# ChristianSteger/HORAYZON

Measured on AMD Instinct MI355X. Metric: grid_cells_per_s (horizon_gridded, 360 azimuths, 3601^2 SRTM-like tile), higher is better.
Workload: dtype f32

## Files before the change

### horayzon_amd/csrc/hz_api.hip

```cpp
#include "hz_internal.h"
#include <cmath>
#include <cstring>
#include <cstdlib>
#include <string>
#include <vector>
#include <limits>
#include <mutex>
#include <utility>
#include <thread>
#include <atomic>

namespace hz {

static thread_local std::string g_error;

int set_error(int code, const char *fmt, ...) {
    char buf[1024];
    va_list ap;
    va_start(ap, fmt);
    vsnprintf(buf, sizeof(buf), fmt, ap);
    va_end(ap);
    g_error = buf;
    return code;
}
// ... 400 lines not shown
    if (hipEventCreate(&n0) != hipSuccess || hipEventCreate(&n1) != hipSuccess) {
        if (n0) (void)hipEventDestroy(n0);
        return set_error(HZ_ERR_HIP, "hipEventCreate failed");
    }
    (void)hipEventRecord(n0, st);
    const int rc = near_launch(sc, na, st);
    (void)hipEventRecord(n1, st);
    if (!rc) {
        (void)hipEventSynchronize(n1);
        float mn = 0.0f;
        (void)hipEventElapsedTime(&mn, n0, n1);
        *ms_near += mn;
    }
    (void)hipEventDestroy(n0); (void)hipEventDestroy(n1);
    return rc;
}

static int plan_leftover(const Scene *sc, const hz_opts *opts, int rows_max, int dim_in_1, int left_t[HZ_LEFT_LEVELS], HorizonArgs &a) {
    int n_left_launches = 0;
    for (int l = 0; l < HZ_LEFT_LEVELS; l++) left_t[l] = 0;
    const int pack = opts ? opts->left_min : 0;
    const unsigned upack = pack == 0 ? HZ_LEFT_DEFAULT : (pack < 0 ? 0u : (unsigned)pack);
    for (int l = 0; l < HZ_LEFT_LEVELS; l++) {
        left_t[l] = (int)std::min((upack >> (8 * l)) & 0xffu, 56u);
        if (left_t[l] == 0) break;
        n_left_launches = l + 1;
    }
    if ((opts && opts->count_work) || n_left_launches == 0) return 0;
    const TileMap tm = make_tile_map((rows_max + 15) / 16, (dim_in_1 + 15) / 16);
    unsigned long long units = (unsigned long long)tm.per_xcd * 8ull * 4ull;
    unsigned long long total = 0, cap_max = 0;
    for (int l = 0; l < n_left_launches; l++) {
        unsigned long long cap = ((units * (unsigned long long)left_t[l] + 63ull) & ~63ull) + 64ull;
        if (opts && opts->left_cap_test > 0) cap = std::min<unsigned long long>(cap, ((unsigned long long)opts->left_cap_test + 63ull) & ~63ull);
        a.left_base[l] = (unsigned)total; a.left_cap[l] = (unsigned)cap;
        total += cap; cap_max = std::max(cap_max, cap);
        units = cap / 64ull;
    }
    const size_t rec_bytes = (size_t)total * HZ_LEFT_WORDS * sizeof(unsigned);
    const size_t sort_words = 4 * (size_t)cap_max + sort_temp_elems((size_t)cap_max) + 64;
    const size_t need = rec_bytes + sort_words * sizeof(uint32_t);
    if (total >= (1ull << 31) || (unsigned long long)rows_max * (unsigned long long)dim_in_1 >= 0xffffffffull) return 0;
    if (sc->left_bytes < need) {
        if (sc->left_buf) (void)hipFree(sc->left_buf);
        sc->left_buf = nullptr; sc->left_bytes = 0;
        if (hipMalloc(&sc->left_buf, need) != hipSuccess) { (void)hipGetLastError(); sc->left_buf = nullptr; return 0; }
        sc->left_bytes = need;
// ... 117 lines not shown
    a.mid_idx = d_mid.dev;
    a.top_nodes = opts ? opts->top_nodes : -1;
    a.regroup = opts ? opts->regroup : -1;
    a.count_work = opts ? opts->count_work : 0;
    a.hit_cache = (opts && opts->no_hit_cache) ? 0 : 1;
    a.counters = (unsigned long long *)cnt_dev;
    const int near_opt = opts ? opts->no_near_skip : 0;
    const bool height_field = (sc->hdr.flags & HZ_BLOB_HEIGHT_FIELD) != 0;
    const bool bad_map = (sc->hdr.flags & HZ_BLOB_BAD_MAP) != 0;
    const bool use_near = near_opt <= 0 && (height_field || bad_map || near_opt < 0) &&
                          azim_num <= near_max_azim() && tb.elev_num <= 65534;
    a.near_idx = nullptr; a.near_r = nullptr; a.scratch_row = nullptr;
    a.tile_list = nullptr; a.n_list = 0;
    const int verify_n = (opts && opts->verify_near > 0) ? opts->verify_near : 0;
    a.verify_near = (opts && opts->count_work) ? verify_n : 0;
    float ms_near = 0.0f;

    unsigned long long cnt[16] = {0}, n_verified = 0, n_mon_violations = 0;
    NearMonitor mon;
    float ms = 0.0f, ms_svf = 0.0f;
    int fallbacks = 0;
    unsigned long long redo_blocks = 0, redo_groups = 0;

    struct Ev { hipEvent_t a = nullptr, b = nullptr, c = nullptr, d = nullptr, l = nullptr; };
    std::vector<Ev> evs;
    std::vector<size_t> ev_of;
    hipStream_t st_copy = nullptr;
    auto free_events = [&]() {
        for (auto &e : evs) {
            if (e.a) (void)hipEventDestroy(e.a);
            if (e.b) (void)hipEventDestroy(e.b);
            if (e.c) (void)hipEventDestroy(e.c);
            if (e.d) (void)hipEventDestroy(e.d);
            if (e.l) (void)hipEventDestroy(e.l);
        }
        if (st_copy) { stream_release(sc->device, st_copy); st_copy = nullptr; }
    };
    if (stream_out && (rc = stream_acquire(sc->device, &st_copy))) return rc;
    if (use_near) {
        const size_t cells = (size_t)std::min(chunk_rows, row_end - row_begin) * dim_in_1;
        const size_t need = ((cells * (size_t)azim_num * 2 + 255) & ~(size_t)255) + cells * 4;
        if (sc->near_bytes < need) {
            if (sc->near_buf) (void)hipFree(sc->near_buf);
            sc->near_buf = nullptr; sc->near_bytes = 0;
            if (hipMalloc(&sc->near_buf, need) != hipSuccess) { free_events(); return set_error(HZ_ERR_HIP, "hipMalloc of the near-field certificates failed"); }
            sc->near_bytes = need;
        }
    }
    int left_t[HZ_LEFT_LEVELS];
    const int n_left_launches = plan_leftover(sc, opts, std::min(chunk_rows, row_end - row_begin), dim_in_1, left_t, a);
    a.left_min = n_left_launches > 0 ? left_t[0] : 0;
    a.left_rec = n_left_launches > 0 ? (unsigned *)sc->left_buf : nullptr;
    a.left_regroup = (opts && (opts->left_tune & 0xff) > 0) ? (opts->left_tune & 0xff) : HZ_LEFT_REGROUP;
    a.left_key_shift = (opts && ((opts->left_tune >> 8) & 0xff) > 0) ? std::min(((opts->left_tune >> 8) & 0xff) - 1, 8) : HZ_LEFT_KEY_SHIFT;
    a.persist_grid = (opts && opts->persist_grid > 0) ? opts->persist_grid : 0;
    a.no_persist = (opts && opts->persist_grid < 0) ? 1 : 0;
    unsigned *near_reasons = nullptr;
    struct ReasonsFree { unsigned **p; ~ReasonsFree() { if (*p) (void)hipFree(*p); } } reasons_free{&near_reasons};
    if (use_near && opts && opts->verbose >= 2) {
        if (hipMalloc((void **)&near_reasons, 20 * sizeof(unsigned)) != hipSuccess) { (void)hipGetLastError(); near_reasons = nullptr; }
        else (void)hipMemsetAsync(near_reasons, 0, 20 * sizeof(unsigned), st);
    }
    HostPinner pinner;
    if (stream_out && !(opts && opts->no_host_pin)) {
        std::vector<size_t> cb;
        for (int rb = row_begin; rb < row_end; rb += chunk_rows) cb.push_back((size_t)(std::min(rb + chunk_rows, row_end) - rb) * row_bytes);
        pinner.start(sc->device, reinterpret_cast<char *>(hori_slab_host), cb);
    }
    auto copy_out = [&](int k) -> int {
        const int rb = row_begin + k * chunk_rows, re = std::min(rb + chunk_rows, row_end);
        const void *src = (k & 1) ? tmp_hori2 : tmp_hori;
        Ev &e = evs[ev_of[(size_t)k]];
        char *dst = reinterpret_cast<char *>(hori_row0 + (size_t)rb * dim_in_1 * azim_num);
        const size_t bytes = (size_t)(re - rb) * row_bytes;
        std::vector<size_t> cuts;
        if (!pinner.planned.empty()) cuts = pinner.cuts_for(dst, bytes);
        cuts.push_back(bytes);
// ... 35 lines not shown
        }
        {
            Ev e;
            if (hipEventCreate(&e.a) != hipSuccess || hipEventCreate(&e.b) != hipSuccess || hipEventCreate(&e.c) != hipSuccess ||
                hipEventCreate(&e.d) != hipSuccess) {
                evs.push_back(e);
                return fail(set_error(HZ_ERR_HIP, "hipEventCreate failed"));
            }
            evs.push_back(e);
            ev_of.push_back(evs.size() - 1);
            if (hipMemcpyAsync(cnt_dev, zeros, sizeof(zeros), hipMemcpyHostToDevice, st) != hipSuccess)
                return fail(set_error(HZ_ERR_HIP, "counter reset failed"));
            if (stream_out && n_chunk >= 2) (void)hipStreamWaitEvent(st, evs[ev_of[(size_t)n_chunk - 2]].d, 0);
            a.level_stack = (sc->level_stack.load(std::memory_order_relaxed) != 0 || (opts && opts->level_stack > 0)) ? 1
                            : ((opts && opts->level_stack < 0) ? opts->level_stack : 0);
            (void)hipEventRecord(e.a, st);
            if (verify_n > 0 && !a.count_work && use_near) {
                if ((rc = mon.launch(sc, a, verify_n, rb, st))) return fail(rc);
            }
            auto launch_chunk = [&](int *safe_out) -> int {
                int r = horizon_launch(sc, a, st, safe_out);
                if (r || n_left_launches == 0) return r;
                if (!evs.back().l && hipEventCreate(&evs.back().l) != hipSuccess) return set_error(HZ_ERR_HIP, "hipEventCreate failed");
                (void)hipEventRecord(evs.back().l, st);
                for (int l = 1; l <= n_left_launches && !r; l++) {
                    if ((r = left_sort(a, l - 1, st))) break;
                    HorizonArgs b = a;
                    b.left_mode = l; b.left_min = l < n_left_launches ? left_t[l] : 0;
                    if (n_left_launches > 1) b.level_stack = 1;
                    b.tile_list = nullptr; b.n_list = 0;
                    r = horizon_launch(sc, b, st, nullptr);
                }
                return r;
            };
            int safe = 0;
            rc = launch_chunk(&safe);
            if (!rc && !safe) {
                unsigned long long cov[32] = {0};
                if (hipMemcpyAsync(cov, cnt_dev, sizeof(cov), hipMemcpyDeviceToHost, st) != hipSuccess ||
                    hipStreamSynchronize(st) != hipSuccess)
                    return fail(set_error(HZ_ERR_HIP, "horizon kernel failed: %s", hipGetErrorString(hipGetLastError())));
                const unsigned long long ov = cov[8], lov = cov[30];
                if (ov != 0 || lov != 0) {
                    const unsigned long long tiles = (unsigned long long)((re - rb + 7) / 8) * (unsigned long long)((dim_in_1 + 7) / 8);
                    fallbacks++;
                    a.level_stack = 1;
                    if (ov <= HZ_REDO_CAP && lov <= HZ_REDO_CAP && (ov + lov) * 4 <= tiles) {
                        redo_blocks += ov + lov; redo_groups += lov;
                        if (ov != 0) {
                            a.tile_list = reinterpret_cast<const int *>((unsigned long long *)cnt_dev + HZ_CNT_N);
                            a.n_list = (int)ov;
                            rc = horizon_launch(sc, a, st, &safe);
                            a.tile_list = nullptr; a.n_list = 0;
                        }
                        if (!rc && lov != 0) {
                            HorizonArgs b = a;
                            b.left_mode = 1; b.left_min = 0;
                            b.tile_list = reinterpret_cast<const int *>((unsigned long long *)cnt_dev + HZ_CNT_N) + HZ_REDO_CAP;
                            b.n_list = (int)lov;
                            rc = horizon_launch(sc, b, st, nullptr);
                        }
                    } else {
                        sc->level_stack.store(1, std::memory_order_relaxed);
                        if (hipMemcpyAsync(cnt_dev, zeros, sizeof(zeros), hipMemcpyHostToDevice, st) != hipSuccess)
                            return fail(set_error(HZ_ERR_HIP, "counter reset failed"));
                        (void)hipEventRecord(e.a, st);
                        rc = launch_chunk(&safe);
                    }
                }
            }
            if (!rc && mon.active) rc = mon.collect(st, &n_verified, &n_mon_violations);
            (void)hipEventRecord(e.b, st);
            if (!rc && want_topo) {
                const size_t o = (size_t)(rb - row_begin) * dim_in_1;
                const float *tilt_chunk = tilt0 ? tilt0 + 3 * (size_t)rb * dim_in_1 : nullptr;
                if (!want_vsf && !want_open)
                    rc = svf_launch(d_azim.dev, hori_chunk, tilt_chunk, re - rb, dim_in_1, azim_num, d_svf.dev + o, st);
                else
                    rc = topo_multi_launch(d_azim.dev, hori_chunk, tilt_chunk, re - rb, dim_in_1, azim_num,
                                           want_svf ? d_svf.dev + o : nullptr, want_vsf ? d_vsf.dev + o : nullptr,
                                           want_open ? d_open.dev + o : nullptr, st);
            }
            (void)hipEventRecord(e.c, st);
            if (!rc && stream_out && n_chunk >= 1) rc = copy_out(n_chunk - 1);
            if (rc) return fail(rc);
            unsigned long long c[HZ_CNT_N];
            if (hipMemcpyAsync(c, cnt_dev, sizeof(c), hipMemcpyDeviceToHost, st) != hipSuccess ||
                hipStreamSynchronize(st) != hipSuccess)
                return fail(set_error(HZ_ERR_HIP, "horizon kernel failed: %s", hipGetErrorString(hipGetLastError())));
            float m1 = 0.0f, m2 = 0.0f;
            (void)hipEventElapsedTime(&m1, e.a, e.b);
            (void)hipEventElapsedTime(&m2, e.b, e.c);
            ms += m1; ms_svf += m2;
            if (evs.back().l) { float m3 = 0.0f; (void)hipEventElapsedTime(&m3, evs.back().l, e.b); ms_left += m3; }
            for (int k = 0; k < 16; k++) cnt[k] += c[k];
            left_cells += c[28]; left_again += c[29];
            n_verified += c[21];
            if (a.count_work && opts && opts->verbose >= 3) {
                const unsigned long long t0 = ~c[20];
                fprintf(stderr, "hz xcd spans [ms] rows %d..%d:", rb, re);
                for (int x = 0; x < 8; x++) fprintf(stderr, " %.1f", c[12 + x] ? (double)(c[12 + x] - t0) * 1.0e-5 : 0.0);
                fprintf(stderr, "\n");
            }
        }
    }
    Timer t_d2h; t_d2h.start();
    if (stream_out) {
        rc = copy_out(n_chunk - 1);
        const hipError_t se = hipStreamSynchronize(st_copy);
        pinner.finish();
        if (!rc && se != hipSuccess) rc = set_error(HZ_ERR_HIP, "copy of the horizon failed: %s", hipGetErrorString(se));
        if (rc) { free_events(); return rc; }
    }
    free_events();
    HZ_HIP(hipGetLastError());
    if ((rc = d_hori.finish(st))) return rc;
    if ((rc = d_svf.finish(st))) return rc;
// ... 423 lines not shown
    const size_t bytes = (n ? n : 1) * 4;
    HZ_HIP(hipMalloc(&di, bytes)); HZ_HIP(hipMalloc(&dout, bytes)); HZ_HIP(hipMalloc(&tmp, scan_temp_elems(n) * 4 + 16));
    HZ_HIP(hipMemcpy(di, in, n * 4, hipMemcpyHostToDevice));
    rc = exclusive_scan_u32((const uint32_t *)di, (uint32_t *)dout, n, (uint32_t *)tmp, st);
    if (!rc) {
        HZ_HIP(hipStreamSynchronize(st));
        HZ_HIP(hipMemcpy(out, dout, n * 4, hipMemcpyDeviceToHost));
    }
    (void)hipFree(di); (void)hipFree(dout); (void)hipFree(tmp);
    return rc;
}

int hz_debug_valu_peak(int device, int packed, int waves_per_simd, double *winst_per_s_per_simd,
                       double *clock_ghz, int *simds) {
    int rc = select_device(device);
    if (rc) return rc;
    return bench_valu_peak(packed, waves_per_simd, winst_per_s_per_simd, clock_ghz, simds);
}

int hz_debug_set(const char *key, int value) {
    if (!key) return hz::set_error(HZ_ERR_ARG, "hz_debug_set: null key");
    if (!strcmp(key, "shadow_fast_cap")) hz::g_shadow_fast_cap.store(value < 0 ? HZ_SHADOW_FAST_CAP_DEFAULT : value, std::memory_order_relaxed);
    else if (!strcmp(key, "topo_wide")) hz::g_topo_wide.store(value != 0, std::memory_order_relaxed);
    else if (!strcmp(key, "accum_chunk")) hz::g_accum_chunk.store(value < 0 ? 0 : value, std::memory_order_relaxed);
    else return hz::set_error(HZ_ERR_ARG, "hz_debug_set: unknown key '%s'", key);
    return HZ_OK;
}

int hz_debug_inst_rate(int device, int op, double *cycles_per_inst) {
    int rc = select_device(device);
    if (rc) return rc;
    return bench_inst_rate(op, cycles_per_inst);
}

int hz_debug_copy_peak(int device, size_t bytes, double *gbs) {
    int rc = select_device(device);
    if (rc) return rc;
    return bench_copy_peak(bytes, gbs);
}

static int slope_api(int which, const float *x, const float *y, const float *z, int len_0, int len_1,
                     const float *rot_mat, int output_rot, float *vec_tilt, int device) {
    if (!x || !y || !z || !vec_tilt) return set_error(HZ_ERR_ARG, "NULL argument");
    if (len_0 <= 0 || len_1 <= 0) return set_error(HZ_ERR_ARG, "Inconsistent shapes / number of dimensions of input arrays");
    if (which == 1 && output_rot && !rot_mat) return set_error(HZ_ERR_ARG, "'rot_mat' must be provided for 'output_rot = True'");
    int rc = select_device(device);
// ... 544 lines not shown
```

### horayzon_amd/csrc/hz_horizon.hip

```cpp
#include "hz_search.h"
#include <vector>

namespace hz {

#ifndef HZ_TPB
#define HZ_TPB 256
#endif
#define HZ_WPB (HZ_TPB / 64)
#ifndef HZ_QLEN
#define HZ_QLEN 2
#endif

struct HorizonParams {
    SceneView sv;
    Tables tb;
    const float *vec_norm, *vec_north;
    const uint8_t *mask;
    float *hori;
    int offset_0, offset_1, dim_in_1;
    int row_begin, row_end;
    TileMap tm;
    float dist, hori_fill, ray_org_elev;
    float dist_box, neg_tau;
    int top_nodes, regroup, stack_bytes, leaf_bias, stage_bytes, hit_cache, stack_cap;
    int pre_bytes;
    const unsigned short *near_idx;
    const float *near_r;
    float *scratch_row;
    int verify_near;
    unsigned verify_mask;
    unsigned long long *counters;
    const int *tile_list;
    int n_list;
    int *redo_list;
    int left_min, left_mode;
    unsigned left_in_base;
    unsigned left_out_base, left_out_cap;
    unsigned *left_rec, *left_in_ctl, *left_out_ctl;
    const unsigned *left_perm;
    int persist;
    unsigned *queue;
};

__device__ __forceinline__ void hz_left_write(unsigned *w, unsigned cert, unsigned k, unsigned flags,
                                                        unsigned ind, unsigned prev, unsigned pazim, unsigned count, float lim_up, float lim_low,
                                                        float elev_samp, float ev, unsigned cache, float st0, float st1, float st2) {
    w[0] = cert;
    w[1] = k; w[2] = flags; w[3] = ind; w[4] = prev; w[5] = pazim; w[6] = count;
    w[7] = __float_as_uint(lim_up); w[8] = __float_as_uint(lim_low); w[9] = __float_as_uint(elev_samp); w[10] = __float_as_uint(ev);
    w[11] = cache; w[12] = __float_as_uint(st0); w[13] = __float_as_uint(st1); w[14] = __float_as_uint(st2); w[15] = 0u;
}

template <int ALG, bool COUNT, bool STAGE, bool NODELET, bool LEVELSTACK, bool LEFT = false>
#ifndef HZ_WG_PER_CU
#define HZ_WG_PER_CU 5
#endif
__global__ __launch_bounds__(HZ_TPB, (COUNT ? 4 : HZ_WG_PER_CU) * (4 / HZ_WPB)) void k_horizon(HorizonParams p_arg) {
    typedef const __attribute__((address_space(4))) HorizonParams *hz_kparams;
    hz_kparams pk = (hz_kparams)__builtin_amdgcn_kernarg_segment_ptr();
#if defined(__HIP_DEVICE_COMPILE__)
#define HZ_LOAD_PARAMS(dst) dst = *pk
#else
#define HZ_LOAD_PARAMS(dst) dst = p_arg
#endif
    HorizonParams p;
    HZ_LOAD_PARAMS(p);
    extern __shared__ __attribute__((aligned(16))) unsigned char smem[];
    int *stack = reinterpret_cast<int *>(smem + p.pre_bytes);
    const float4 *top = reinterpret_cast<const float4 *>(smem + p.pre_bytes + p.stack_bytes);
    const int tid = threadIdx.x;
    const int ntop = p.top_nodes;
    if (NODELET && ntop > 0) {
        float4 *dst = reinterpret_cast<float4 *>(smem + p.pre_bytes + p.stack_bytes);
        const float4 *src = reinterpret_cast<const float4 *>(p.sv.nodes);
        for (int i = tid; i < ntop * 2; i += HZ_TPB) dst[i] = src[i];
        __syncthreads();
    }

    const int wave = __builtin_amdgcn_readfirstlane(tid >> 6);
    const int xcc_own = (int)(__builtin_amdgcn_s_getreg((3 << 11) | 20) & 7u);
    int xcc_off = 0;
    int left_on = 1;
  for (;;) {
    asm volatile("" : "+s"(pk));
    HZ_LOAD_PARAMS(p);
    int tid_b = tid;
    asm volatile("" : "+v"(tid_b));
    const int lane = tid_b & 63;
#define HZ_KEEP(x) asm volatile("" : "+s"(x))
    HZ_KEEP(p.leaf_bias); HZ_KEEP(p.regroup); HZ_KEEP(p.neg_tau); HZ_KEEP(p.sv.cx); HZ_KEEP(p.sv.cy); HZ_KEEP(p.sv.cz);
    HZ_KEEP(p.near_idx); HZ_KEEP(p.near_r);
#undef HZ_KEEP
    int ti = 0, tj = 0;
    int blk = (int)blockIdx.x * HZ_WPB + wave;
    unsigned rec0 = 0u, rec_n = 0u;
    if (LEFT) {
        blk = -1;
        const unsigned groups = (p.left_in_ctl[1] + 63u) / 64u;
        if (p.tile_list) {
            const int b = (int)blockIdx.x * HZ_WPB + wave;
            const int g = b < p.n_list ? p.tile_list[b] : -1;
            if (g >= 0 && (unsigned)g < groups) { blk = g; rec0 = (unsigned)g * 64u; rec_n = min(64u, p.left_in_ctl[1] - (unsigned)g * 64u); }
        } else
        while (xcc_off < 8) {
            const unsigned x = (unsigned)((xcc_own + xcc_off) & 7);
            unsigned q = 0u;
            if (lane == 0) q = atomicAdd(&p.left_in_ctl[8 + x], 1u);
            q = (unsigned)__builtin_amdgcn_readfirstlane((int)q);
            const unsigned g = (((q >> 5) * 8u + x) << 5) | (q & 31u);
            if (g < groups) { blk = (int)g; rec0 = g * 64u; rec_n = min(64u, p.left_in_ctl[1] - g * 64u); break; }
            xcc_off++;
        }
        if (blk < 0) break;
    } else if (p.persist) {
        blk = -1;
        while (xcc_off < 8) {
            const int x = (xcc_own + xcc_off) & 7;
            int q = 0;
            if (lane == 0) q = (int)atomicAdd(&p.queue[x], 1u);
            q = __builtin_amdgcn_readfirstlane(q);
            if (q < p.tm.per_xcd * 4) { blk = (((q >> 2) * 8 + x) << 2) | (q & 3); break; }
            xcc_off++;
        }
        if (blk < 0) break;
    } else if (p.tile_list) blk = (blk < p.n_list) ? p.tile_list[blk] : -1;
    else if (HZ_WPB != 4) {
        const int b = (int)blockIdx.x, x = b & 7, t = b >> 3, per = 4 / HZ_WPB;
        blk = (((t / per) * 8 + x) * 4) + (t % per) * HZ_WPB + wave;
    }
    blk = __builtin_amdgcn_readfirstlane(blk);
    bool has_tile = blk >= 0 && (LEFT || hz_tile_of_block(p.tm, blk >> 2, &ti, &tj));
    int i = p.row_begin + ti * 16 + ((blk >> 1) & 1) * 8 + (lane >> 3);
    int j = tj * 16 + (blk & 1) * 8 + (lane & 7);
    const unsigned *rec = nullptr;
    if (LEFT) {
        has_tile = (unsigned)lane < rec_n;
        if (has_tile) {
            rec = p.left_rec + ((size_t)p.left_in_base + (size_t)p.left_perm[rec0 + (unsigned)lane]) * HZ_LEFT_WORDS;
            const unsigned c0 = rec[0];
            has_tile = c0 != 0xffffffffu;
            const unsigned di = c0 / (unsigned)p.dim_in_1;
            i = p.row_begin + (int)di; j = (int)(c0 - di * (unsigned)p.dim_in_1);
        }
    }
    const bool in_dom = has_tile && (i < p.row_end) && (j < p.dim_in_1);

    const Tables &t = p.tb;
    const unsigned long long t_start = COUNT ? (unsigned long long)wall_clock64() : 0ull;
    const size_t cell = in_dom ? ((size_t)i * p.dim_in_1 + j) : 0;
    bool done = !in_dom;
    const unsigned cert = in_dom ? (unsigned)(i - p.row_begin) * (unsigned)p.dim_in_1 + (unsigned)j : 0u;
    const bool to_scratch = COUNT && p.scratch_row != nullptr;
    float *const hori0 = to_scratch ? p.scratch_row : p.hori + (size_t)p.row_begin * p.dim_in_1 * (size_t)t.azim_num;
    const unsigned cell_stride = to_scratch ? 0u : 1u;
    Sink out;
    out.hori = COUNT ? hori0 + (size_t)(cert * cell_stride) * (size_t)t.azim_num : hori0 + (size_t)cert * (size_t)t.azim_num;
    out.dist = nullptr; out.dist_hit = 0.0f;
    out.stage = reinterpret_cast<float *>(smem) + tid_b;
    out.stride = HZ_TPB;
    float ox = 0, oy = 0, oz = 0;
    float r01 = 0, r02 = 0, r11 = 0, r12 = 0, r21 = 0, r22 = 0;
    const bool masked = in_dom && p.mask[cell] != 1;
    {
        unsigned long long m = __ballot(masked);
        while (m) {
            const int src = __ffsll((long long)m) - 1;
            m &= m - 1;
            float *row = COUNT ? hori0 + (size_t)((unsigned)__shfl((int)cert, src) * cell_stride) * (size_t)t.azim_num
                               : hori0 + (size_t)__shfl((int)cert, src) * (size_t)t.azim_num;
            for (int k = lane; k < t.azim_num; k += 64) row[k] = p.hori_fill;
        }
    }
    if (in_dom) {
        if (masked) {
// ... 34 lines not shown
    float tn = 0.0f;
    bool had_guard = false;
    if (LEFT && !done) {
        s.k = (int)rec[1]; s.phase = (int)(rec[2] & 0xffu); s.ind = (int)rec[3]; s.prev = (int)rec[4]; s.pazim = (int)rec[5]; s.count = (int)rec[6];
        s.lim_up = __uint_as_float(rec[7]); s.lim_low = __uint_as_float(rec[8]); s.elev_samp = __uint_as_float(rec[9]); s.ev = __uint_as_float(rec[10]);
        cache = (int)rec[11];
        last_hit = (rec[2] & 0x100u) != 0u;
        had_guard = (rec[2] & 0x400u) != 0u;
        if (STAGE) { out.stage[0] = __uint_as_float(rec[12]); out.stage[out.stride] = __uint_as_float(rec[13]); out.stage[2 * out.stride] = __uint_as_float(rec[14]); }
        if (rec[2] & 0x200u) {
            const float ec = t.elev_cos[s.ind], es = t.elev_sin[s.ind];
            const float rx = ec * t.azim_sin[s.k], ry = ec * t.azim_cos[s.k], rz = es;
            const float r00 = r11 * r22 - r21 * r12, r10 = r21 * r02 - r01 * r22, r20 = r01 * r12 - r11 * r02;
            dx = (r00 * rx + r01 * ry) + r02 * rz;
            dy = (r10 * rx + r11 * ry) + r12 * rz;
            dz = (r20 * rx + r21 * ry) + r22 * rz;
            HZ_OC(ocx, ocy, ocz)
            rb = hz_raybox(ocx + p.neg_tau * dx, ocy + p.neg_tau * dy, ocz + p.neg_tau * dz, dx, dy, dz);
            hz_trav_reset(ts);
            ray_active = true;
        }
    }

    int left_min = (COUNT || !left_on || __popcll(__ballot(!done)) <= p.left_min + 8) ? 0 : p.left_min;
    while (__ballot(!done) != 0ull) {
        if (!COUNT && left_min > 0 && __popcll(__ballot(!done)) <= left_min) {
            const unsigned long long um = __ballot(!done);
            if (um != 0ull && !(!LEVELSTACK && __ballot(overflow) != 0ull)) {
                const unsigned n = (unsigned)__popcll(um);
                unsigned *const out_rec = p.left_rec + (size_t)p.left_out_base * HZ_LEFT_WORDS;
                unsigned base = 0u;
                if (lane == 0) base = atomicAdd(&p.left_out_ctl[0], n);
                base = (unsigned)__builtin_amdgcn_readfirstlane((int)base);
                if (base + n > p.left_out_cap) {
                    left_on = 0; left_min = 0;
                    if (base + (unsigned)lane < p.left_out_cap) out_rec[(size_t)(base + (unsigned)lane) * HZ_LEFT_WORDS] = 0xffffffffu;
                } else {
                    if (lane == 0) atomicAdd(&p.counters[LEFT ? 29 : 28], (unsigned long long)n);
                    if (!done) {
                        const unsigned rank = (unsigned)__builtin_amdgcn_mbcnt_hi((unsigned)(um >> 32), __builtin_amdgcn_mbcnt_lo((unsigned)um, 0u));
                        const unsigned flags = (unsigned)s.phase | (last_hit ? 0x100u : 0u) | (ray_active ? 0x200u : 0u) | ((guards != 0u || had_guard) ? 0x400u : 0u);
                        hz_left_write(out_rec + (size_t)(base + rank) * HZ_LEFT_WORDS, cert, (unsigned)s.k, flags,
                                      (unsigned)s.ind, (unsigned)s.prev, (unsigned)s.pazim, (unsigned)s.count, s.lim_up, s.lim_low, s.elev_samp, s.ev, (unsigned)cache,
                                      STAGE ? out.stage[0] : 0.0f, STAGE ? out.stage[out.stride] : 0.0f, STAGE ? out.stage[2 * out.stride] : 0.0f);
                        done = true;
                    }
                }
            }
// ... 43 lines not shown
        bool start_v = false, viol = false;
        if (ray_active) {
            int r;
            r = hz_trace<HZ_TPB, COUNT, HZ_QLEN, NODELET, LEVELSTACK>(p.sv.nodes, p.sv.prims, top, ntop, stack, tid, ox, oy, oz,
                                                 dx, dy, dz, tfar, p.dist_box, rb, ts, p.regroup, p.leaf_bias, tc, p.stack_cap, overflow);
            if (r == 0 && second) {
                second = false; hz_trav_reset(ts);
            } else if (COUNT && want_v && r != 2) {
                want_v = false; verifying = true; first_result = (r == 1); start_v = true;
                HZ_OC(ocx, ocy, ocz)
                rb = hz_raybox(ocx + p.neg_tau * dx, ocy + p.neg_tau * dy, ocz + p.neg_tau * dz, dx, dy, dz);
                hz_trav_reset(ts);
            } else if (r != 2) {
                if (COUNT && verifying) { viol = ((r == 1) != first_result); verifying = false; }
                ray_active = false; last_hit = (r == 1);
                if (r == 1) cache = p.sv.anc[HZ_LEAF_ID(ts.lq0)];
            }
        }
        if (COUNT) {
            w_verified += (unsigned)__popcll(__ballot(start_v));
            w_violations += (unsigned)__popcll(__ballot(viol));
        }
    }
    unsigned long long r = rays, g = guards, nc = tc.nodes, tcn = tc.tris, cc = cells_cnt;
    unsigned long long wn = tc.w_nodes, wl = tc.w_leaves, wa = w_adv;
    for (int off = 32; off > 0; off >>= 1) {
        r += __shfl_xor(r, off); g += __shfl_xor(g, off); cc += __shfl_xor(cc, off);
        if (COUNT) {
            nc += __shfl_xor(nc, off); tcn += __shfl_xor(tcn, off);
            wn += __shfl_xor(wn, off); wl += __shfl_xor(wl, off); wa += __shfl_xor(wa, off);
        }
    }
    const bool wave_overflowed = !LEVELSTACK && __ballot(overflow) != 0ull;
    if (wave_overflowed) {
        if (lane == 0) {
            const unsigned long long slot = atomicAdd(&p.counters[LEFT ? 30 : 8], 1ull);
            if (slot < (unsigned long long)HZ_REDO_CAP) p.redo_list[(LEFT ? HZ_REDO_CAP : 0) + (int)slot] = blk;
        }
    } else {
    const int guard_cells = __popcll(__ballot(guards != 0u && !(LEFT && had_guard)));
    if (lane == 0) {
        if (r) atomicAdd(&p.counters[0], r);
        if (g) { atomicAdd(&p.counters[1], g); atomicAdd(&p.counters[11], (unsigned long long)guard_cells); }
        if (cc) atomicAdd(&p.counters[4], cc);
        if (COUNT) {
            atomicAdd(&p.counters[2], nc); atomicAdd(&p.counters[3], tcn);
            atomicAdd(&p.counters[5], wn); atomicAdd(&p.counters[6], wl); atomicAdd(&p.counters[7], wa);
        }
    }
    if (COUNT) {
        if (lane == 0) {
            const unsigned xcc = __builtin_amdgcn_s_getreg((3 << 11) | 20) & 7u;
            atomicMax(&p.counters[12 + xcc], (unsigned long long)wall_clock64());
            atomicMax(&p.counters[20], ~t_start);
        }
    }
    if (COUNT) {
        unsigned long long sh = shortened;
        for (int off = 32; off > 0; off >>= 1) sh += __shfl_xor(sh, off);
        if (lane == 0) {
            if (sh) atomicAdd(&p.counters[9], sh);
            if (w_violations) atomicAdd(&p.counters[10], (unsigned long long)w_violations);
            if (w_verified) atomicAdd(&p.counters[21], (unsigned long long)w_verified);
        }
    }
    }
    if (!p.persist) break;
  }
}

static long long resident_workgroups(const void *func, size_t lds) {
    struct Key { const void *f; size_t lds; int dev; long long n; };
    static std::mutex mu;
    static std::vector<Key> cache;
    int dev = 0;
    if (hipGetDevice(&dev) != hipSuccess) { (void)hipGetLastError(); return 0; }
    std::lock_guard<std::mutex> lock(mu);
    for (const Key &k : cache) if (k.f == func && k.lds == lds && k.dev == dev) return k.n;
    int per_cu = 0;
    hipDeviceProp_t prop;
    long long n = 0;
    if (hipOccupancyMaxActiveBlocksPerMultiprocessor(&per_cu, func, HZ_TPB, lds) == hipSuccess && per_cu > 0 &&
        hipGetDeviceProperties(&prop, dev) == hipSuccess && prop.multiProcessorCount > 0)
        n = (long long)per_cu * prop.multiProcessorCount;
    else (void)hipGetLastError();
    cache.push_back(Key{func, lds, dev, n});
    return n;
}

template <int ALG, bool COUNT, bool STAGE, bool NODELET, bool LEVELSTACK>
static int launch_one(const HorizonParams &p_in, int grid, size_t lds, int persist_grid, hipStream_t st) {
    const void *func = reinterpret_cast<const void *>(k_horizon<ALG, COUNT, STAGE, NODELET, LEVELSTACK>);
    HZ_HIP(hipFuncSetAttribute(func, hipFuncAttributeMaxDynamicSharedMemorySize, (int)lds));
    HorizonParams p = p_in;
    if (p.persist) {
        const long long resident = persist_grid > 0 ? (long long)persist_grid : resident_workgroups(func, lds);
        if (resident <= 0 || (long long)grid <= resident) p.persist = 0;
        else {
            grid = (int)resident;
            HZ_HIP(hipMemsetAsync(p.queue, 0, 8 * sizeof(unsigned), st));
        }
    }
    hipLaunchKernelGGL((k_horizon<ALG, COUNT, STAGE, NODELET, LEVELSTACK>), dim3(grid), dim3(HZ_TPB), lds, st, p);
    HZ_HIP(hipGetLastError());
    return HZ_OK;
}

template <int ALG, bool STAGE, bool LS>
static int launch_left(const HorizonParams &p, size_t lds, int persist_grid, hipStream_t st) {
    const void *func = reinterpret_cast<const void *>(k_horizon<ALG, false, STAGE, false, LS, true>);
    HZ_HIP(hipFuncSetAttribute(func, hipFuncAttributeMaxDynamicSharedMemorySize, (int)lds));
    long long grid = p.tile_list ? (long long)((p.n_list + HZ_WPB - 1) / HZ_WPB)
                                 : (persist_grid > 0 ? (long long)persist_grid : resident_workgroups(func, lds));
    if (grid <= 0) grid = 1024;
    hipLaunchKernelGGL((k_horizon<ALG, false, STAGE, false, LS, true>), dim3((unsigned)grid), dim3(HZ_TPB), lds, st, p);
    HZ_HIP(hipGetLastError());
    return HZ_OK;
}

__device__ __forceinline__ unsigned hz_spread16(unsigned v) {
    v &= 0xffffu; v = (v | (v << 8)) & 0x00ff00ffu; v = (v | (v << 4)) & 0x0f0f0f0fu; v = (v | (v << 2)) & 0x33333333u; v = (v | (v << 1)) & 0x55555555u;
    return v;
}
__global__ __launch_bounds__(256) void k_left_keys(const unsigned *__restrict__ rec, unsigned cap, unsigned *__restrict__ ctl, unsigned dim_in_1,
                                                   unsigned azim_num, int morton_shift, int class_shift, unsigned *__restrict__ keys,
                                                   unsigned *__restrict__ vals) {
    const unsigned idx = blockIdx.x * 256u + threadIdx.x;
    const unsigned cnt = min(ctl[0], cap);
    bool valid = false;
    unsigned key = 0x00ffffffu;
    if (idx < cnt) {
        const unsigned c = rec[(size_t)idx * HZ_LEFT_WORDS];
        if (c != 0xffffffffu) {
            valid = true;
            const unsigned k = rec[(size_t)idx * HZ_LEFT_WORDS + 1];
// ... 87 lines not shown
    top = std::min(top, std::max(0, (80 * 1024 - (p.stack_bytes + p.pre_bytes)) / (int)sizeof(Node)));
    top = std::min(top, sc->hdr.n_top);
    p.top_nodes = top;
    p.regroup = (a.regroup <= 0) ? 36 : std::min(a.regroup & 0xff, 64);
    if (a.left_mode && a.left_regroup > 0) p.regroup = std::min(a.left_regroup, 64);
    p.leaf_bias = (a.regroup >= 256) ? (a.regroup >> 8) : 24;
    p.hit_cache = (a.hit_cache != 0) ? 1 : 0;
    p.near_idx = a.near_idx; p.near_r = a.near_r;
    p.verify_near = (a.verify_near > 0 && a.near_idx != nullptr) ? 1 : 0;
    p.scratch_row = a.count_work ? a.scratch_row : nullptr;
    {
        unsigned n = a.verify_near > 1 ? (unsigned)a.verify_near : 1u, m = 1u;
        while (m < n && m < (1u << 30)) m <<= 1;
        p.verify_mask = m - 1u;
    }
    p.counters = a.counters;
    p.tile_list = a.tile_list; p.n_list = a.n_list;
    p.redo_list = reinterpret_cast<int *>(a.counters + HZ_CNT_N);
    p.left_mode = std::max(a.left_mode, 0);
    p.left_rec = a.left_rec;
    unsigned *const left_ctl = reinterpret_cast<unsigned *>(a.counters + HZ_CNT_LEFT);
    const bool hands_over = a.left_rec != nullptr && !a.tile_list && !a.count_work && a.left_min > 0 && p.left_mode < HZ_LEFT_LEVELS &&
                            a.left_cap[p.left_mode] >= 64u;
    p.left_min = hands_over ? std::min(a.left_min, 56) : 0;
    p.left_in_base = p.left_mode ? a.left_base[p.left_mode - 1] : 0u;
    p.left_perm = (p.left_mode && a.left_sort) ? a.left_sort + 3 * a.left_cap_max : nullptr;
    p.left_in_ctl = left_ctl + 16 * (p.left_mode ? p.left_mode - 1 : 0);
    p.left_out_base = hands_over ? a.left_base[p.left_mode] : 0u;
    p.left_out_cap = hands_over ? a.left_cap[p.left_mode] : 0u;
    p.left_out_ctl = left_ctl + 16 * std::min(p.left_mode, HZ_LEFT_LEVELS - 1);
    p.persist = (a.tile_list == nullptr && ((!a.no_persist && HZ_WPB == 4) || p.left_mode)) ? 1 : 0;
    p.queue = reinterpret_cast<unsigned *>(a.counters + 24);
    const size_t lds = (size_t)p.pre_bytes + (size_t)p.stack_bytes + (size_t)top * sizeof(Node);
    const int grid = a.tile_list ? (a.n_list + HZ_WPB - 1) / HZ_WPB : p.tm.per_xcd * 8 * (4 / HZ_WPB);
    if (grid <= 0) return HZ_OK;
    const bool count = a.count_work != 0;
    int rc_launch;
    switch (a.alg) {
        case ALG_DISCRETE: rc_launch = launch_alg<ALG_DISCRETE>(p, grid, lds, count, level_stack, a.persist_grid, st); break;
        case ALG_BINARY: rc_launch = launch_alg<ALG_BINARY>(p, grid, lds, count, level_stack, a.persist_grid, st); break;
        default: rc_launch = launch_alg<ALG_GUESS>(p, grid, lds, count, level_stack, a.persist_grid, st); break;
    }
    return rc_launch;
}

__device__ __forceinline__ void hz_sincos_halfpi_f(float x, float &s, float &c) {
    const float y = 0.5f * x, z = y * y;
// ... 319 lines not shown
```

### horayzon_amd/csrc/hz_internal.h

```cpp
#pragma once
#include <hip/hip_runtime.h>
#include <algorithm>
#include <chrono>
#include <cstdarg>
#include <cstdio>
#include <cstdlib>
#include "../../include/horayzon_hip.h"
#include "hz_common.h"
#include <atomic>
#include <mutex>

#define HZ_MAX_TOP_NODES 2047
#define HZ_MAX_STACK 40
#ifndef HZ_ANC_LEVELS
#define HZ_ANC_LEVELS 4
#endif

namespace hz {

int set_error(int code, const char *fmt, ...);

#define HZ_SHADOW_FAST_CAP_DEFAULT 19
extern std::atomic<int> g_shadow_fast_cap;
extern std::atomic<int> g_topo_wide;
extern std::atomic<int> g_accum_chunk;

#define HZ_HIP(expr)                                                                      \
    do {                                                                                  \
        hipError_t e_ = (expr);                                                           \
        if (e_ != hipSuccess)                                                             \
            return ::hz::set_error(HZ_ERR_HIP, "%s failed: %s (%s:%d)", #expr,            \
                                   hipGetErrorString(e_), __FILE__, __LINE__);            \
    } while (0)

struct Timer {
    std::chrono::high_resolution_clock::time_point t0;
    void start() { t0 = std::chrono::high_resolution_clock::now(); }
    double stop() const {
        return std::chrono::duration<double>(std::chrono::high_resolution_clock::now() - t0).count();
    }
};

struct Scene {
    int device = 0;
    hipStream_t stream = nullptr;
    void *blob = nullptr;
    size_t blob_bytes = 0;
// ... 54 lines not shown
struct HorizonArgs {
    const float *vec_norm, *vec_north;
    const uint8_t *mask;
    float *hori;
    int offset_0, offset_1, dim_in_0, dim_in_1;
    int row_begin, row_end;
    int azim_num, elev_num, alg;
    float hori_acc, low, up, dist;
    float hori_fill, ray_org_elev;
    const float *azim_sin, *azim_cos, *elev_ang, *elev_sin, *elev_cos;
    const int *mid_idx;
    int top_nodes, regroup, count_work, hit_cache;
    int level_stack;
    const int *tile_list;
    int n_list;
    const unsigned short *near_idx;
    const float *near_r;
    int verify_near;
    float *scratch_row;
    int left_min = 0;
    unsigned *left_rec = nullptr;
    int left_mode = 0;
    unsigned left_base[HZ_LEFT_LEVELS] = {0, 0, 0, 0}, left_cap[HZ_LEFT_LEVELS] = {0, 0, 0, 0};
    int left_regroup = 0, left_key_shift = 0;
    uint32_t *left_sort = nullptr;
    unsigned left_cap_max = 0;
    int no_persist = 0;
    int persist_grid = 0;
    unsigned long long *counters;
};
#define HZ_LEFT_DEFAULT 0x00000024u
#define HZ_LEFT_KEY_SHIFT 3
#define HZ_LEFT_REGROUP 24
#define HZ_CNT_LEFT 32
#define HZ_CNT_N 64
#define HZ_LEFT_WORDS 16
#define HZ_REDO_CAP 16384
int horizon_launch(const Scene *sc, const HorizonArgs &a, hipStream_t st, int *used_level_stack = nullptr);
int left_sort(const HorizonArgs &a, int region, hipStream_t st);
int horizon_num_blocks(const HorizonArgs &a);
int topo_launch(int kind, const float *azim, const float *hori, const float *vec_tilt, int len_0, int len_1,
                int len_2, float *out, hipStream_t st);
int svf_launch(const float *azim, const float *hori, const float *vec_tilt, int len_0, int len_1,
               int len_2, float *svf, hipStream_t st);
int topo_multi_launch(const float *azim, const float *hori, const float *vec_tilt, int len_0, int len_1, int len_2,
                      float *svf, float *vsf, float *openness, hipStream_t st);

struct NearArgs {
    const float *vec_norm, *vec_north;
    const uint8_t *mask;
    const float *azim_sin, *azim_cos;
    int offset_0, offset_1, dim_in_1, row_begin, row_end, azim_num, elev_num;
    float ray_org_elev, hori_acc, low, up;
    unsigned short *near_idx;
    float *near_r;
    unsigned *reasons = nullptr;
// ... 83 lines not shown
```

Baseline: 9.940 million.

## Stream leftover cells into freed wave lanes with per-lane state save and refill

Reworks the leftover (LEFT) kernel so that a wave no longer takes a fixed group of 64 records. When enough lanes finish, it breaks out, saves the unfinished lanes' ray-traversal state to per-lane registers, and refills the free lanes from a shared record cursor. Overflow redo moves to per-cell granularity through a cell-position list. The streaming path is gated behind a debug flag that is off by default, but the per-lane redo, the tally changes and the left_min cap change (56 to 55) apply unconditionally. The added state save and restore code may raise register pressure and lower occupancy.

```diff
diff --git a/horayzon_amd/csrc/hz_api.hip b/horayzon_amd/csrc/hz_api.hip
--- a/horayzon_amd/csrc/hz_api.hip
+++ b/horayzon_amd/csrc/hz_api.hip
@@ -446,7 +446,7 @@
     const int pack = opts ? opts->left_min : 0;
     const unsigned upack = pack == 0 ? HZ_LEFT_DEFAULT : (pack < 0 ? 0u : (unsigned)pack);
     for (int l = 0; l < HZ_LEFT_LEVELS; l++) {
-        left_t[l] = (int)std::min((upack >> (8 * l)) & 0xffu, 56u);
+        left_t[l] = (int)std::min((upack >> (8 * l)) & 0xffu, (unsigned)HZ_LEFT_MIN_MAX);
         if (left_t[l] == 0) break;
         n_left_launches = l + 1;
     }
@@ -610,7 +610,7 @@
     int fallbacks = 0;
     unsigned long long redo_blocks = 0, redo_groups = 0;
 
-    struct Ev { hipEvent_t a = nullptr, b = nullptr, c = nullptr, d = nullptr, l = nullptr; };
+    struct Ev { hipEvent_t a = nullptr, b = nullptr, c = nullptr, d = nullptr, l = nullptr, m = nullptr; };
     std::vector<Ev> evs;
     std::vector<size_t> ev_of;
     hipStream_t st_copy = nullptr;
@@ -621,6 +621,7 @@
             if (e.c) (void)hipEventDestroy(e.c);
             if (e.d) (void)hipEventDestroy(e.d);
             if (e.l) (void)hipEventDestroy(e.l);
+            if (e.m) (void)hipEventDestroy(e.m);
         }
         if (st_copy) { stream_release(sc->device, st_copy); st_copy = nullptr; }
     };
@@ -641,6 +642,7 @@
     a.left_rec = n_left_launches > 0 ? (unsigned *)sc->left_buf : nullptr;
     a.left_regroup = (opts && (opts->left_tune & 0xff) > 0) ? (opts->left_tune & 0xff) : HZ_LEFT_REGROUP;
     a.left_key_shift = (opts && ((opts->left_tune >> 8) & 0xff) > 0) ? std::min(((opts->left_tune >> 8) & 0xff) - 1, 8) : HZ_LEFT_KEY_SHIFT;
+    a.left_refill = g_left_stream.load(std::memory_order_relaxed) ? g_left_refill.load(std::memory_order_relaxed) : 0;
     a.persist_grid = (opts && opts->persist_grid > 0) ? opts->persist_grid : 0;
     a.no_persist = (opts && opts->persist_grid < 0) ? 1 : 0;
     unsigned *near_reasons = nullptr;
@@ -722,6 +724,7 @@
                 int r = horizon_launch(sc, a, st, safe_out);
                 if (r || n_left_launches == 0) return r;
                 if (!evs.back().l && hipEventCreate(&evs.back().l) != hipSuccess) return set_error(HZ_ERR_HIP, "hipEventCreate failed");
+                if (!evs.back().m && hipEventCreate(&evs.back().m) != hipSuccess) return set_error(HZ_ERR_HIP, "hipEventCreate failed");
                 (void)hipEventRecord(evs.back().l, st);
                 for (int l = 1; l <= n_left_launches && !r; l++) {
                     if ((r = left_sort(a, l - 1, st))) break;
@@ -731,6 +734,7 @@
                     b.tile_list = nullptr; b.n_list = 0;
                     r = horizon_launch(sc, b, st, nullptr);
                 }
+                (void)hipEventRecord(evs.back().m, st);
                 return r;
             };
             int safe = 0;
@@ -740,13 +744,13 @@
                 if (hipMemcpyAsync(cov, cnt_dev, sizeof(cov), hipMemcpyDeviceToHost, st) != hipSuccess ||
                     hipStreamSynchronize(st) != hipSuccess)
                     return fail(set_error(HZ_ERR_HIP, "horizon kernel failed: %s", hipGetErrorString(hipGetLastError())));
-                const unsigned long long ov = cov[8], lov = cov[30];
+                const unsigned long long ov = cov[8], lov = cov[30], lgr = (lov + 63ull) / 64ull;
                 if (ov != 0 || lov != 0) {
                     const unsigned long long tiles = (unsigned long long)((re - rb + 7) / 8) * (unsigned long long)((dim_in_1 + 7) / 8);
                     fallbacks++;
                     a.level_stack = 1;
-                    if (ov <= HZ_REDO_CAP && lov <= HZ_REDO_CAP && (ov + lov) * 4 <= tiles) {
-                        redo_blocks += ov + lov; redo_groups += lov;
+                    if (ov <= HZ_REDO_CAP && lov <= HZ_REDO_CAP && (ov + lgr) * 4 <= tiles) {
+                        redo_blocks += ov + lgr; redo_groups += lgr;
                         if (ov != 0) {
                             a.tile_list = reinterpret_cast<const int *>((unsigned long long *)cnt_dev + HZ_CNT_N);
                             a.n_list = (int)ov;
@@ -792,7 +796,7 @@
             (void)hipEventElapsedTime(&m1, e.a, e.b);
             (void)hipEventElapsedTime(&m2, e.b, e.c);
             ms += m1; ms_svf += m2;
-            if (evs.back().l) { float m3 = 0.0f; (void)hipEventElapsedTime(&m3, evs.back().l, e.b); ms_left += m3; }
+            if (evs.back().l && evs.back().m) { float m3 = 0.0f; (void)hipEventElapsedTime(&m3, evs.back().l, evs.back().m); ms_left += m3; }
             for (int k = 0; k < 16; k++) cnt[k] += c[k];
             left_cells += c[28]; left_again += c[29];
             n_verified += c[21];
@@ -1262,6 +1266,8 @@
     if (!key) return hz::set_error(HZ_ERR_ARG, "hz_debug_set: null key");
     if (!strcmp(key, "shadow_fast_cap")) hz::g_shadow_fast_cap.store(value < 0 ? HZ_SHADOW_FAST_CAP_DEFAULT : value, std::memory_order_relaxed);
     else if (!strcmp(key, "topo_wide")) hz::g_topo_wide.store(value != 0, std::memory_order_relaxed);
+    else if (!strcmp(key, "left_stream")) hz::g_left_stream.store(value != 0, std::memory_order_relaxed);
+    else if (!strcmp(key, "left_refill")) hz::g_left_refill.store(value <= 0 ? HZ_LEFT_REFILL : std::min(value, 64), std::memory_order_relaxed);
     else if (!strcmp(key, "accum_chunk")) hz::g_accum_chunk.store(value < 0 ? 0 : value, std::memory_order_relaxed);
     else return hz::set_error(HZ_ERR_ARG, "hz_debug_set: unknown key '%s'", key);
     return HZ_OK;
diff --git a/horayzon_amd/csrc/hz_horizon.hip b/horayzon_amd/csrc/hz_horizon.hip
--- a/horayzon_amd/csrc/hz_horizon.hip
+++ b/horayzon_amd/csrc/hz_horizon.hip
@@ -2,6 +2,9 @@
 #include <vector>
 
 namespace hz {
+
+std::atomic<int> g_left_stream{0};
+std::atomic<int> g_left_refill{HZ_LEFT_REFILL};
 
 #ifndef HZ_TPB
 #define HZ_TPB 256
@@ -36,6 +39,7 @@
     int left_min, left_mode;
     unsigned left_in_base;
     unsigned left_out_base, left_out_cap;
+    int left_refill;
     unsigned *left_rec, *left_in_ctl, *left_out_ctl;
     const unsigned *left_perm;
     int persist;
@@ -81,6 +85,10 @@
     const int xcc_own = (int)(__builtin_amdgcn_s_getreg((3 << 11) | 20) & 7u);
     int xcc_off = 0;
     int left_on = 1;
+    unsigned ls_cur = 0u, ls_end = 0u;
+    int ls_exhausted = 0;
+    bool c_done = true;
+    volatile unsigned cs[42];
   for (;;) {
     asm volatile("" : "+s"(pk));
     HZ_LOAD_PARAMS(p);
@@ -93,25 +101,39 @@
 #undef HZ_KEEP
     int ti = 0, tj = 0;
     int blk = (int)blockIdx.x * HZ_WPB + wave;
-    unsigned rec0 = 0u, rec_n = 0u;
+    bool take = true;
+    unsigned pos = 0u;
     if (LEFT) {
-        blk = -1;
-        const unsigned groups = (p.left_in_ctl[1] + 63u) / 64u;
+        blk = 0;
+        const unsigned n_valid = p.left_in_ctl[1];
+        const unsigned groups = (n_valid + 63u) / 64u;
+        const unsigned long long free_m = __ballot(c_done);
         if (p.tile_list) {
             const int b = (int)blockIdx.x * HZ_WPB + wave;
-            const int g = b < p.n_list ? p.tile_list[b] : -1;
-            if (g >= 0 && (unsigned)g < groups) { blk = g; rec0 = (unsigned)g * 64u; rec_n = min(64u, p.left_in_ctl[1] - (unsigned)g * 64u); }
-        } else
-        while (xcc_off < 8) {
-            const unsigned x = (unsigned)((xcc_own + xcc_off) & 7);
-            unsigned q = 0u;
-            if (lane == 0) q = atomicAdd(&p.left_in_ctl[8 + x], 1u);
-            q = (unsigned)__builtin_amdgcn_readfirstlane((int)q);
-            const unsigned g = (((q >> 5) * 8u + x) << 5) | (q & 31u);
-            if (g < groups) { blk = (int)g; rec0 = g * 64u; rec_n = min(64u, p.left_in_ctl[1] - g * 64u); break; }
-            xcc_off++;
-        }
-        if (blk < 0) break;
+            take = b * 64 + lane < p.n_list;
+            if (take) pos = (unsigned)p.tile_list[b * 64 + lane];
+            take = take && pos < n_valid;
+            ls_exhausted = 1;
+        } else {
+            if (ls_cur >= ls_end && !ls_exhausted) {
+                ls_exhausted = 1;
+                while (xcc_off < 8) {
+                    const unsigned x = (unsigned)((xcc_own + xcc_off) & 7);
+                    unsigned q = 0u;
+                    if (lane == 0) q = atomicAdd(&p.left_in_ctl[8 + x], 1u);
+                    q = (unsigned)__builtin_amdgcn_readfirstlane((int)q);
+                    const unsigned g = (((q >> 5) * 8u + x) << 5) | (q & 31u);
+                    if (g < groups) { ls_cur = g * 64u; ls_end = ls_cur + min(64u, n_valid - g * 64u); ls_exhausted = 0; break; }
+                    xcc_off++;
+                }
+            }
+            const unsigned n_take = min((unsigned)__popcll(free_m), ls_end - ls_cur);
+            const unsigned rank = (unsigned)__builtin_amdgcn_mbcnt_hi((unsigned)(free_m >> 32), __builtin_amdgcn_mbcnt_lo((unsigned)free_m, 0u));
+            take = c_done && rank < n_take;
+            pos = ls_cur + rank;
+            ls_cur = (unsigned)__builtin_amdgcn_readfirstlane((int)(ls_cur + n_take));
+        }
+        if (ls_exhausted && __ballot(take) == 0ull && free_m == ~0ull) break;
     } else if (p.persist) {
         blk = -1;
         while (xcc_off < 8) {
@@ -134,14 +156,15 @@
     int j = tj * 16 + (blk & 1) * 8 + (lane & 7);
     const unsigned *rec = nullptr;
     if (LEFT) {
-        has_tile = (unsigned)lane < rec_n;
+        has_tile = take;
         if (has_tile) {
-            rec = p.left_rec + ((size_t)p.left_in_base + (size_t)p.left_perm[rec0 + (unsigned)lane]) * HZ_LEFT_WORDS;
+            rec = p.left_rec + ((size_t)p.left_in_base + (size_t)p.left_perm[pos]) * HZ_LEFT_WORDS;
             const unsigned c0 = rec[0];
             has_tile = c0 != 0xffffffffu;
             const unsigned di = c0 / (unsigned)p.dim_in_1;
             i = p.row_begin + (int)di; j = (int)(c0 - di * (unsigned)p.dim_in_1);
         }
+        if (!LEVELSTACK && take) reinterpret_cast<unsigned *>(smem + p.pre_bytes - HZ_TPB * 4)[tid_b] = pos;
     }
     const bool in_dom = has_tile && (i < p.row_end) && (j < p.dim_in_1);
 
@@ -149,7 +172,7 @@
     const unsigned long long t_start = COUNT ? (unsigned long long)wall_clock64() : 0ull;
     const size_t cell = in_dom ? ((size_t)i * p.dim_in_1 + j) : 0;
     bool done = !in_dom;
-    const unsigned cert = in_dom ? (unsigned)(i - p.row_begin) * (unsigned)p.dim_in_1 + (unsigned)j : 0u;
+    unsigned cert = in_dom ? (unsigned)(i - p.row_begin) * (unsigned)p.dim_in_1 + (unsigned)j : 0u;
     const bool to_scratch = COUNT && p.scratch_row != nullptr;
     float *const hori0 = to_scratch ? p.scratch_row : p.hori + (size_t)p.row_begin * p.dim_in_1 * (size_t)t.azim_num;
     const unsigned cell_stride = to_scratch ? 0u : 1u;
@@ -230,8 +253,29 @@
         }
     }
 
-    int left_min = (COUNT || !left_on || __popcll(__ballot(!done)) <= p.left_min + 8) ? 0 : p.left_min;
+    if (LEFT && !take && !c_done) {
+        done = false;
+        cert = cs[0]; rays = cs[1]; guards = cs[2];
+        const unsigned fl = cs[3];
+        ray_active = (fl & 1u) != 0u; last_hit = (fl & 2u) != 0u; second = (fl & 4u) != 0u; overflow = (fl & 8u) != 0u; had_guard = (fl & 16u) != 0u;
+#define HZ_CF(k) __uint_as_float(cs[k])
+        ox = HZ_CF(4); oy = HZ_CF(5); oz = HZ_CF(6); r01 = HZ_CF(7); r02 = HZ_CF(8); r11 = HZ_CF(9); r12 = HZ_CF(10); r21 = HZ_CF(11); r22 = HZ_CF(12);
+        dx = HZ_CF(13); dy = HZ_CF(14); dz = HZ_CF(15);
+        s.k = (int)cs[16]; s.phase = (int)cs[17]; s.ind = (int)cs[18]; s.prev = (int)cs[19]; s.pazim = (int)cs[20]; s.count = (int)cs[21];
+        s.lim_up = HZ_CF(22); s.lim_low = HZ_CF(23); s.elev_samp = HZ_CF(24); s.ev = HZ_CF(25);
+        rb.rdx = HZ_CF(26); rb.rdy = HZ_CF(27); rb.rdz = HZ_CF(28); rb.ordx = HZ_CF(29); rb.ordy = HZ_CF(30); rb.ordz = HZ_CF(31);
+        rb.sel_x = cs[32]; rb.sel_y = cs[33]; rb.sel_z = cs[34];
+        ts.node = (int)cs[35]; ts.sp = (int)cs[36]; ts.pf = (int)cs[37]; ts.pm = (int)cs[38]; ts.lq0 = (int)cs[39]; ts.lq1 = (int)cs[40];
+        cache = (int)cs[41];
+#undef HZ_CF
+    }
+    const bool ls_stream = LEFT && p.left_refill > 0 && !p.tile_list;
+    int refill_n = (ls_stream && !ls_exhausted) ? min(max(p.left_refill, 1), 64) : 65;
+    if (LEFT) asm volatile("" : "+s"(refill_n));
+
+    int left_min = (COUNT || !left_on || (ls_stream ? !ls_exhausted : __popcll(__ballot(!done)) <= p.left_min + 8)) ? 0 : p.left_min;
     while (__ballot(!done) != 0ull) {
+        if (LEFT && __popcll(__ballot(done)) >= refill_n) break;
         if (!COUNT && left_min > 0 && __popcll(__ballot(!done)) <= left_min) {
             const unsigned long long um = __ballot(!done);
             if (um != 0ull && !(!LEVELSTACK && __ballot(overflow) != 0ull)) {
@@ -321,7 +365,19 @@
             w_violations += (unsigned)__popcll(__ballot(viol));
         }
     }
-    unsigned long long r = rays, g = guards, nc = tc.nodes, tcn = tc.tris, cc = cells_cnt;
+    if (LEFT && !LEVELSTACK) {
+        const unsigned long long om = __ballot(done && overflow);
+        if (om != 0ull) {
+            unsigned long long slot = 0ull;
+            if (lane == 0) slot = atomicAdd(&p.counters[30], (unsigned long long)__popcll(om));
+            slot = (unsigned long long)(unsigned)__builtin_amdgcn_readfirstlane((int)(unsigned)slot);
+            const unsigned rank = (unsigned)__builtin_amdgcn_mbcnt_hi((unsigned)(om >> 32), __builtin_amdgcn_mbcnt_lo((unsigned)om, 0u));
+            if (done && overflow && slot + rank < (unsigned long long)HZ_REDO_CAP)
+                p.redo_list[HZ_REDO_CAP + (int)slot + (int)rank] = (int)reinterpret_cast<unsigned *>(smem + p.pre_bytes - HZ_TPB * 4)[tid_b];
+        }
+    }
+    const bool tally = !LEFT || (done && !(!LEVELSTACK && overflow));
+    unsigned long long r = tally ? rays : 0u, g = tally ? guards : 0u, nc = tc.nodes, tcn = tc.tris, cc = cells_cnt;
     unsigned long long wn = tc.w_nodes, wl = tc.w_leaves, wa = w_adv;
     for (int off = 32; off > 0; off >>= 1) {
         r += __shfl_xor(r, off); g += __shfl_xor(g, off); cc += __shfl_xor(cc, off);
@@ -330,14 +386,14 @@
             wn += __shfl_xor(wn, off); wl += __shfl_xor(wl, off); wa += __shfl_xor(wa, off);
         }
     }
-    const bool wave_overflowed = !LEVELSTACK && __ballot(overflow) != 0ull;
+    const bool wave_overflowed = !LEFT && !LEVELSTACK && __ballot(overflow) != 0ull;
     if (wave_overflowed) {
         if (lane == 0) {
-            const unsigned long long slot = atomicAdd(&p.counters[LEFT ? 30 : 8], 1ull);
-            if (slot < (unsigned long long)HZ_REDO_CAP) p.redo_list[(LEFT ? HZ_REDO_CAP : 0) + (int)slot] = blk;
+            const unsigned long long slot = atomicAdd(&p.counters[8], 1ull);
+            if (slot < (unsigned long long)HZ_REDO_CAP) p.redo_list[(int)slot] = blk;
         }
     } else {
-    const int guard_cells = __popcll(__ballot(guards != 0u && !(LEFT && had_guard)));
+    const int guard_cells = __popcll(__ballot(tally && guards != 0u && !(LEFT && had_guard)));
     if (lane == 0) {
         if (r) atomicAdd(&p.counters[0], r);
         if (g) { atomicAdd(&p.counters[1], g); atomicAdd(&p.counters[11], (unsigned long long)guard_cells); }
@@ -363,6 +419,23 @@
             if (w_verified) atomicAdd(&p.counters[21], (unsigned long long)w_verified);
         }
     }
+    }
+    if (LEFT) {
+        c_done = done;
+        if (!done) {
+            cs[0] = cert; cs[1] = rays; cs[2] = guards;
+            cs[3] = (ray_active ? 1u : 0u) | (last_hit ? 2u : 0u) | (second ? 4u : 0u) | (overflow ? 8u : 0u) | (had_guard ? 16u : 0u);
+#define HZ_CU(x) __float_as_uint(x)
+            cs[4] = HZ_CU(ox); cs[5] = HZ_CU(oy); cs[6] = HZ_CU(oz); cs[7] = HZ_CU(r01); cs[8] = HZ_CU(r02); cs[9] = HZ_CU(r11); cs[10] = HZ_CU(r12);
+            cs[11] = HZ_CU(r21); cs[12] = HZ_CU(r22); cs[13] = HZ_CU(dx); cs[14] = HZ_CU(dy); cs[15] = HZ_CU(dz);
+            cs[16] = (unsigned)s.k; cs[17] = (unsigned)s.phase; cs[18] = (unsigned)s.ind; cs[19] = (unsigned)s.prev; cs[20] = (unsigned)s.pazim;
+            cs[21] = (unsigned)s.count; cs[22] = HZ_CU(s.lim_up); cs[23] = HZ_CU(s.lim_low); cs[24] = HZ_CU(s.elev_samp); cs[25] = HZ_CU(s.ev);
+            cs[26] = HZ_CU(rb.rdx); cs[27] = HZ_CU(rb.rdy); cs[28] = HZ_CU(rb.rdz); cs[29] = HZ_CU(rb.ordx); cs[30] = HZ_CU(rb.ordy); cs[31] = HZ_CU(rb.ordz);
+            cs[32] = rb.sel_x; cs[33] = rb.sel_y; cs[34] = rb.sel_z;
+            cs[35] = (unsigned)ts.node; cs[36] = (unsigned)ts.sp; cs[37] = (unsigned)ts.pf; cs[38] = (unsigned)ts.pm; cs[39] = (unsigned)ts.lq0;
+            cs[40] = (unsigned)ts.lq1; cs[41] = (unsigned)cache;
+#undef HZ_CU
+        }
     }
     if (!p.persist) break;
   }
@@ -409,7 +482,7 @@
 static int launch_left(const HorizonParams &p, size_t lds, int persist_grid, hipStream_t st) {
     const void *func = reinterpret_cast<const void *>(k_horizon<ALG, false, STAGE, false, LS, true>);
     HZ_HIP(hipFuncSetAttribute(func, hipFuncAttributeMaxDynamicSharedMemorySize, (int)lds));
-    long long grid = p.tile_list ? (long long)((p.n_list + HZ_WPB - 1) / HZ_WPB)
+    long long grid = p.tile_list ? (long long)(((p.n_list + 63) / 64 + HZ_WPB - 1) / HZ_WPB)
                                  : (persist_grid > 0 ? (long long)persist_grid : resident_workgroups(func, lds));
     if (grid <= 0) grid = 1024;
     hipLaunchKernelGGL((k_horizon<ALG, false, STAGE, false, LS, true>), dim3((unsigned)grid), dim3(HZ_TPB), lds, st, p);
@@ -543,7 +616,8 @@
     unsigned *const left_ctl = reinterpret_cast<unsigned *>(a.counters + HZ_CNT_LEFT);
     const bool hands_over = a.left_rec != nullptr && !a.tile_list && !a.count_work && a.left_min > 0 && p.left_mode < HZ_LEFT_LEVELS &&
                             a.left_cap[p.left_mode] >= 64u;
-    p.left_min = hands_over ? std::min(a.left_min, 56) : 0;
+    p.left_min = hands_over ? std::min(a.left_min, HZ_LEFT_MIN_MAX) : 0;
+    p.left_refill = (p.left_mode && !a.tile_list) ? std::min(std::max(a.left_refill, 0), 64) : 0;
     p.left_in_base = p.left_mode ? a.left_base[p.left_mode - 1] : 0u;
     p.left_perm = (p.left_mode && a.left_sort) ? a.left_sort + 3 * a.left_cap_max : nullptr;
     p.left_in_ctl = left_ctl + 16 * (p.left_mode ? p.left_mode - 1 : 0);
diff --git a/horayzon_amd/csrc/hz_internal.h b/horayzon_amd/csrc/hz_internal.h
--- a/horayzon_amd/csrc/hz_internal.h
+++ b/horayzon_amd/csrc/hz_internal.h
@@ -23,6 +23,8 @@
 #define HZ_SHADOW_FAST_CAP_DEFAULT 19
 extern std::atomic<int> g_shadow_fast_cap;
 extern std::atomic<int> g_topo_wide;
+extern std::atomic<int> g_left_stream;
+extern std::atomic<int> g_left_refill;
 extern std::atomic<int> g_accum_chunk;
 
 #define HZ_HIP(expr)                                                                      \
@@ -123,6 +125,7 @@
     unsigned *left_rec = nullptr;
     int left_mode = 0;
     unsigned left_base[HZ_LEFT_LEVELS] = {0, 0, 0, 0}, left_cap[HZ_LEFT_LEVELS] = {0, 0, 0, 0};
+    int left_refill = 0;
     int left_regroup = 0, left_key_shift = 0;
     uint32_t *left_sort = nullptr;
     unsigned left_cap_max = 0;
@@ -133,6 +136,8 @@
 #define HZ_LEFT_DEFAULT 0x00000024u
 #define HZ_LEFT_KEY_SHIFT 3
 #define HZ_LEFT_REGROUP 24
+#define HZ_LEFT_REFILL 16
+#define HZ_LEFT_MIN_MAX 55
 #define HZ_CNT_LEFT 32
 #define HZ_CNT_N 64
 #define HZ_LEFT_WORDS 16
```

New measurement: 9.625 million. 3.2% lower.
